# vshmyhlo/retinanet-tensorflow

Measured on AMD Instinct MI355X. Metric: train images/sec (MobileNetV2-FPN RetinaNet 512x512, bs=2/GPU), higher is better.
Workload: dtype f32

## Files before the change

include/rn_hip.h:

```cpp
#ifndef RN_HIP_H
#define RN_HIP_H

#include <stddef.h>
#include <stdint.h>

#ifdef __cplusplus
extern "C" {
#endif

typedef void* rn_stream_t;

enum rn_status {
  RN_OK = 0,
  RN_EINVAL = -1,
  RN_EUNSUPPORTED = -2,
  RN_EHIP = -3,
  RN_EWORKSPACE = -4
};

enum rn_act { RN_ACT_NONE = 0, RN_ACT_RELU = 1, RN_ACT_ELU = 2, RN_ACT_RELU6 = 3, RN_ACT_SIGMOID = 4 };
enum rn_loss_mode { RN_LOSS_BCE_DICE = 0, RN_LOSS_FOCAL = 1 };
enum rn_opt { RN_OPT_MOMENTUM = 0, RN_OPT_RMSPROP = 1, RN_OPT_ADAM = 2 };

#define RN_MAX_SEG 16

typedef struct rn_reduce_list rn_reduce_list;

#define RN_API_VERSION 421
int rn_version(void);
const char* rn_last_error(void);

void rn_same_pad(int n, int k, int s, int* out, int* pad_before);

typedef struct rn_conv_seg {
  const float* x;
  const float* wgt;
  const float* bias;
  float* y;
  const float* dy;
  float* dx;
  int32_t n, h, w;
  int32_t cout;
  int32_t x_ld;
// ... 475 lines not shown
  int32_t store_plain;
  rn_mb_rows grows;
  float* planes;
} rn_mb_gout;
size_t rn_mb_pointwise_bwd_rows(int n, int hw, int cin, int cout, int groups, rn_mb_rows* layout);
size_t rn_mb_pointwise_bwd_workspace(int n, int hw, int cin, int cout);
int rn_mb_pointwise_bwd(const float* x, const rn_mb_norm* in, const rn_mb_dy* dy, const float* w, float* dw, const rn_mb_gout* gout,
                        int n, int hw, int cin, int cout, void* workspace, size_t workspace_bytes, rn_stream_t stream,
                        rn_reduce_list* defer);
size_t rn_mb_depthwise_bwd_rows(int n, int h, int w, int c, int stride, int groups, rn_mb_rows* layout);
size_t rn_mb_depthwise_bwd_workspace(int n, int h, int w, int c, int stride);
int rn_mb_depthwise_bwd(const rn_mb_norm* in, const rn_mb_dy* dy, const float* w, float* dw, const rn_mb_gout* gout, int n, int h,
                        int wd, int stride, void* workspace, size_t workspace_bytes, rn_stream_t stream, rn_reduce_list* defer);
int rn_set_mb_dw_taps(int on);
int rn_get_mb_dw_taps(void);

int rn_iou(const float* a, int64_t na, const float* b, int64_t nb, int pairwise, float* out, int32_t* malformed,
           rn_stream_t stream);

int rn_anchor_assign(const float* boxes, const int32_t* class_ids, const int32_t* num_obj, int nimg, int max_obj,
                     const float* anchor_sizes, int num_anchors, int grid_h, int grid_w, int num_classes,
                     float* cls_out, float* reg_out, uint8_t* trainable_out, int32_t* argmax_out,
                     rn_stream_t stream);
#define RN_MAX_LEVELS 8
typedef struct rn_assign_level {
  const float* anchor_sizes;
  int grid_h, grid_w;
  float* cls_out;
  float* reg_out;
  uint8_t* trainable_out;
// ... 99 lines not shown
```

retinanet-tensorflow_amd/_rn.py:

```python
import ctypes as C
import os

import torch

_HERE = os.path.dirname(os.path.abspath(__file__))
LIB_PATH = os.environ.get("RN_LIB_PATH") or os.path.join(_HERE, "librn_hip.so")

MAX_SEG = 16
ACT = {None: 0, "none": 0, "linear": 0, "relu": 1, "elu": 2, "relu6": 3, "sigmoid": 4}
LOSS_MODE = {"bce_dice": 0, "focal": 1}
OPT = {"momentum": 0, "rmsprop": 1, "adam": 2}
OPT_BLOCK = 1024
LR_MAX_BOUNDARIES = 8
LOSS_STATS_HEADER = 8
OPT_F_NORM, OPT_F_LRDEV, OPT_F_EMA, OPT_F_CLIP, OPT_F_ACCUM, OPT_F_GATE = 1, 2, 4, 8, 16, 32
CTL_F_ACCUM, CTL_F_GUARD, CTL_F_LR, CTL_F_EMA = 1, 2, 4, 8
API_VERSION = 421


class RnError(RuntimeError):
    pass


class LrSchedule(C.Structure):
    _fields_ = [("kind", C.c_int32), ("n_boundaries", C.c_int32), ("base_lr", C.c_double), ("warmup_factor", C.c_double),
                ("final_factor", C.c_double), ("decay_factor", C.c_double), ("warmup_steps", C.c_int64), ("total_steps", C.c_int64),
                ("boundaries", C.c_int64 * LR_MAX_BOUNDARIES)]


class StepControl(C.Structure):
    _fields_ = [("features", C.c_uint32), ("optimizer_kind", C.c_int32),
                ("accumulate_steps", C.c_int32), ("micro_dev", C.c_void_p), ("accum_dev", C.c_void_p),
# ... 220 lines not shown
    "rn_group_norm_sync_bytes", "rn_group_norm_workspace", "rn_group_norm_fwd", "rn_group_norm_bwd", "rn_group_norm_plan",
    "rn_act_fwd", "rn_act_bwd", "rn_upsample_add_fwd", "rn_upsample_add_bwd_top",
    "rn_pack_weights_f16", "rn_pack_weights_f16_bytes", "rn_cast_f32_to_f16", "rn_pad_cast_rgb_f16", "rn_conv2d_fwd_f16", "rn_conv2d_f16_fold_rows", "rn_conv2d_fwd_f16_fold", "rn_group_norm_finalize", "rn_group_norm_apply_f16", "rn_group_norm_apply_res_f16", "rn_maxpool_fwd_f16", "rn_maxpool_gn_fwd_f16", "rn_upsample_add_fwd_f16",
    "rn_act_fwd_f16", "rn_flip_width", "rn_dropout", "rn_dropout_strided", "rn_maxpool_fwd", "rn_maxpool_bwd", "rn_maxpool_bwd_arg", "rn_avgpool_fwd", "rn_avgpool_bwd",
    "rn_loss_workspace", "rn_loss_fwd", "rn_loss_bwd",
    "rn_loss_terms_stats_floats", "rn_loss_terms_workspace", "rn_loss_terms_fwd", "rn_loss_terms_bwd",
    "rn_iou", "rn_anchor_assign", "rn_anchor_assign_levels", "rn_anchor_assign_levels_pair", "rn_decode_boxes", "rn_detect_workspace", "rn_detect",
    "rn_boxes_decode", "rn_nms_classwise_workspace", "rn_nms_classwise",
    "rn_optimizer_workspace", "rn_grad_norm_l2reg", "rn_optimizer_update", "rn_counter_add", "rn_add_segs",
    "rn_mb_rows_max", "rn_mb_compact_rows_layout", "rn_mb_compact_rows", "rn_mb_pointwise_rows", "rn_mb_pointwise_fwd", "rn_mb_depthwise_rows", "rn_mb_depthwise_fwd", "rn_mb_apply",
    "rn_mb_resident_sync_bytes", "rn_mb_resident_rows", "rn_mb_resident_fwd", "rn_set_product_mode", "rn_get_product_mode",
    "rn_set_x3_bfrag", "rn_get_x3_bfrag", "rn_x3_bfrag_ok", "rn_x3_bfrag_bytes", "rn_x3_pack_bfrag", "rn_gemm_batched_bfrag", "rn_conv3x3_winograd_gn_u_bytes", "rn_conv3x3_winograd_gn_weights",
    "rn_conv2d_f16_stats_tiles", "rn_group_norm_fwd_f16_tiles",
    "rn_mb_pointwise_bwd_rows", "rn_mb_pointwise_bwd_workspace", "rn_mb_pointwise_bwd",
    "rn_mb_depthwise_bwd_rows", "rn_mb_depthwise_bwd_workspace", "rn_mb_depthwise_bwd", "rn_set_mb_dw_taps", "rn_get_mb_dw_taps",
    "rn_debug_collective_standin", "rn_optimizer_norm_pairs", "rn_norm_reg_finalize",
    "rn_step_control_eval", "rn_grad_norm_partial",
    "rn_train_metrics_workspace", "rn_train_metrics_pass", "rn_train_metrics_fold", "rn_train_metrics_reset",
]


def lib():
    global _lib
    if _lib is None:
        if not os.path.exists(LIB_PATH):
            raise RnError("librn_hip.so not found at %s: build it with "
                          "`make -C retinanet-tensorflow_amd/csrc` (there is no fallback path)" % LIB_PATH)
        L = C.CDLL(LIB_PATH)
        if not hasattr(L, "rn_version") or L.rn_version() != API_VERSION:
            raise RnError("%s reports ABI version %s, these bindings need %d: rebuild it (make -C retinanet-tensorflow_amd/csrc)"
# ... 72 lines not shown
                                          C.c_void_p, C.c_size_t, C.c_void_p, C.c_void_p, C.c_void_p]
        L.rn_wino_gn_rows.argtypes = [C.c_void_p, C.c_int, C.c_int]
        L.rn_winograd_bwd_products_workspace.argtypes = [C.c_int] * 4
        L.rn_winograd_bwd_products.argtypes = [C.c_void_p] * 3 + [C.c_int] * 3 + [C.c_void_p] * 2 + [C.c_int] * 3 + \
                                              [C.c_void_p, C.c_size_t, C.c_void_p, C.c_void_p]
        L.rn_x3_bfrag_ok.argtypes = [C.c_int] * 3
        L.rn_conv2d_f16_stats_tiles.argtypes = [C.c_void_p, C.c_int, C.c_void_p, C.c_void_p]
        L.rn_group_norm_fwd_f16_tiles.argtypes = [C.c_void_p, C.c_int, C.c_void_p, C.c_void_p, C.c_void_p, C.c_void_p, C.c_void_p, C.c_void_p]
        L.rn_conv3x3_winograd_gn_u_bytes.argtypes = [C.c_int] * 3
        L.rn_conv3x3_winograd_gn_weights.argtypes = [C.c_void_p, C.c_int, C.c_int, C.c_int, C.c_void_p, C.c_size_t, C.c_void_p, C.c_void_p]
        L.rn_x3_bfrag_bytes.argtypes = [C.c_int] * 3
        L.rn_x3_pack_bfrag.argtypes = [C.c_void_p, C.c_void_p] + [C.c_int] * 4 + [C.c_void_p]
        L.rn_gemm_batched_bfrag.argtypes = [C.c_void_p] * 3 + [C.c_int] * 5 + [C.c_void_p]
        L.rn_set_x3_bfrag.argtypes = [C.c_int]
        L.rn_set_mb_dw_taps.argtypes = [C.c_int]
        L.rn_conv3x3_winograd_gn.argtypes = [C.c_void_p, C.c_int, C.c_int, C.c_int, C.c_void_p, C.c_void_p, C.c_int, C.c_void_p,
                                             C.c_void_p, C.c_size_t, C.c_void_p, C.c_void_p, C.c_void_p]
        L.rn_conv3x3_winograd_gn_bwd_wgrad.argtypes = [C.c_void_p, C.c_int, C.c_int, C.c_int, C.c_void_p, C.c_int, C.c_int, C.c_void_p, C.c_size_t,
                                                       C.c_void_p, C.c_int, C.c_void_p]
        L.rn_conv3x3_winograd_gn_bwd.argtypes = [C.c_void_p, C.c_int, C.c_int, C.c_int, C.c_void_p, C.c_void_p, C.c_int, C.c_int,
                                                 C.c_void_p, C.c_void_p, C.c_size_t, C.c_void_p, C.c_void_p, C.c_void_p]
        L.rn_conv3x3_winograd_gn_plan.argtypes = [C.c_void_p] + [C.c_int] * 6 + [C.POINTER(WinoGnPlan)]
        L.rn_group_norm_plan.argtypes = [C.c_void_p, C.c_int, C.c_void_p, C.c_int, C.c_size_t, C.POINTER(GnPlan)]
        L.rn_reduce_rows.argtypes = [C.c_void_p, C.c_void_p, C.c_int64, C.c_int, C.c_int, C.c_void_p, C.c_void_p]
        L.rn_conv2d_bias_grad.argtypes = [C.c_void_p, C.c_int, C.c_void_p, C.c_void_p, C.c_void_p, C.c_size_t,
                                          C.c_void_p, C.c_void_p]
        L.rn_group_norm_workspace.argtypes = [C.c_void_p, C.c_int, C.c_void_p]
        L.rn_group_norm_fwd.argtypes = [C.c_void_p, C.c_int, C.c_void_p, C.c_void_p, C.c_void_p, C.c_void_p,
                                        C.c_size_t, C.c_void_p]
        L.rn_group_norm_bwd.argtypes = [C.c_void_p, C.c_int, C.c_void_p, C.c_void_p, C.c_void_p, C.c_void_p,
# ... 242 lines not shown
```

retinanet-tensorflow_amd/csrc/mbconv.hip:

```cpp
#include <type_traits>

#include "mb_common.h"

namespace {


template <int BM, int BN, int WM, int WN, bool NORM, int ACT, int KS, int NST>
__global__ __launch_bounds__(WM* WN * 64 * KS) void mb_pw_fwd_kernel(const PwFwdArgs a) {
  constexpr int TG = WM * WN * 64;
  constexpr bool RES = NORM && ACT != RN_ACT_ELU && ACT != RN_ACT_RELU6 && ACT != RN_ACT_RELU;
  static_assert(TG * KS >= T || !NORM, "the prologue needs 256 threads");
  constexpr int TM = BM / WM / 32, TN = BN / WN / 32;
  constexpr int KQ = BK / 4, A_RPP = TG / KQ, A_PASS = BM / A_RPP;
  constexpr int NQ = BN / 4, B_RPP = TG / NQ, B_PASS = BK / B_RPP;
  static_assert(A_PASS >= 1 && B_PASS >= 1 && BM % A_RPP == 0 && BK % B_RPP == 0, "tile/threads mismatch");
  constexpr int OPF = BM * LDK + BK * BN;
  static_assert(KS * OPF * 4 >= (T + GMAX) * 16 && OPF >= (WM + 1) * BN * 2, "operand tiles double as scratch");
  static_assert(KS == 1 || KS * OPF >= (KS - 1) * TM * TN * 16 * TG, "operand tiles double as the split-K exchange");
  __shared__ __attribute__((aligned(16))) float smem[KS * OPF];
  __shared__ __attribute__((aligned(16))) float tab[NORM ? 2 * KMAX : 4];
  __shared__ float gstat[NORM ? GMAX : 1][2];
  const int tid = threadIdx.x, grp = tid / TG, lt = tid % TG, lane = lt & 63, wave = lt >> 6;
  float* As = smem + grp * OPF;
  float* Bs = As + BM * LDK;
// ... 359 lines not shown
                     fmaf(P.w, g.w, fmaf(R.w, y.w, Q.w)));
}

struct PwBwdArgs {
  int dbg;
  const float* x; NormDev in; int has_in;
  DyDev dy; const float* w; GoutDev go;
  int n, hw, cin, cout;
  int d_tiles_n, dblocks;
  int w_tiles_m, w_tiles_n, chunk, sps;
  float* slab;
  int wfirst;
};
constexpr int pw_lds(int pb) { return 2 * pb * LDK; }

template <int ACT_OUT, int PB, int KS, int NST>
__device__ __forceinline__ void mb_pw_dgrad_body(const PwBwdArgs& a, float* smem_all, float* tabD, float (*gstat)[2], float (*gc)[2], int blk) {
  constexpr int BM = PB, BN = PB, WM = PB / 32, WN = PB / 32, TM = 1, TN = 1, TG = WM * WN * 64;
  constexpr int KQ = BK / 4, RPP = TG / KQ, A_PASS = BM / RPP, B_PASS = BN / RPP;
  const int tid = threadIdx.x, grp = tid / TG, lt = tid % TG, lane = lt & 63, wave = lt >> 6;
  float* As = smem_all + grp * pw_lds(PB);
  float* Bs = As + BM * LDK;
  const int wm = wave / WN, wn = wave % WN;
  const int bid = rn::xcd_remap(blk, a.dblocks);
  const int tile_n = bid % a.d_tiles_n, tile_m = bid / a.d_tiles_n;
  const int KD = a.cout, ND = a.cin, M = a.n * a.hw;
  const int m0 = tile_m * BM, n0 = tile_n * BN;
  const int sample = m0 / a.hw;
  const bool plain = a.dy.dy != nullptr;
  const __amdgpu_buffer_rsrc_t ga = make_rsrc(plain ? a.dy.dy : a.dy.g, (unsigned)M * KD * 4u);
  const __amdgpu_buffer_rsrc_t ya = make_rsrc(plain ? a.dy.dy : a.dy.nd.y, (unsigned)M * KD * 4u);
// ... 29 lines not shown
  const int l31 = lane & 31, half = lane >> 5;
  const int col = n0 + wn * 32 + l31;
  const bool cok = col < ND;
  float o_mean = 0.f, o_rstd = 1.f, o_gam = 1.f, o_bet = 0.f;
  if (go.has_norm && grp == 0) {
    const int cc = cok ? col : 0, og = cc / go.nd.cpg;
    o_mean = go.nd.mean[sample * go.nd.groups + og]; o_rstd = go.nd.rstd[sample * go.nd.groups + og];
    o_gam = go.nd.gamma[cc]; o_bet = go.nd.beta[cc];
  }
#pragma unroll
  for (int st = 0; st < NST; ++st)
    if (st < nit) load_tiles(st, st);
  bool mask = false;
  uint64_t seed = 0;
  if (!plain) {
    dy_table(a.dy, sample, a.hw, 0, KD, smem_all, gstat, gc, tabD, KMAX, gpre, pre, tid);
    mask = a.dy.g_plain && a.dy.nd.drop_rate > 0.f;
    seed = a.dy.nd.seed + (a.dy.nd.seed_dev ? *a.dy.nd.seed_dev : 0ull);
  }
  if (a.dbg == 1) return;
  auto store_tiles = [&](int it, const int st) {
    const int k = (it * KS + grp) * BK + kq * 4;
#pragma unroll
    for (int i = 0; i < A_PASS; ++i) {
      float4 v = ra[st][i];
      if (!plain) {
        if (k < KD) v = dy_of(v, ry[st][i], tabD, KMAX, k, mask, a.dy.nd.drop_rate, a.dy.nd.keep_scale, seed,
                              (uint64_t)(m0 + r0 + i * RPP) * KD + k);
        else v = make_float4(0.f, 0.f, 0.f, 0.f);
      }
      *reinterpret_cast<float4*>(&As[(r0 + i * RPP) * LDK + kq * 4]) = v;
    }
#pragma unroll
    for (int j = 0; j < B_PASS; ++j) *reinterpret_cast<float4*>(&Bs[(r0 + j * RPP) * LDK + kq * 4]) = rb[st][j];
  };
  f32x16 acc[TM][TN];
  zero_acc<TM, TN>(acc);
  for (int it0 = 0; it0 < nit; it0 += NST) {
#pragma unroll
    for (int st = 0; st < NST; ++st) {
      const int it = it0 + st;
      if (it < nit) {
// ... 172 lines not shown
      const int it = it0 + st;
      if (it < nit) {
        store_tiles(it, st);
        __syncthreads();
        if (it + NST < nit) load_tiles(it + NST, st);
        if (it * KS + grp < nk) mma_ktile<BM, BN, WM, WN, true, false>(As, Bs, acc, wm, wn, lane);
        __syncthreads();
      }
    }
  }
  if (a.dbg == 2) { if (acc[0][0][0] == 123.456f) a.slab[0] = 0.f; return; }
  sum_groups<KS, 1, TG>(&acc[0][0], smem_all, grp, lt);
  if (grp == 0) store_tile<BM, BN, WM, WN>(acc, a.slab + (size_t)split * KI * NO, nullptr, m0, n0, KI, NO, NO, wm, wn, lane);
}

template <int ACT_IN, int ACT_OUT, int DPB, int DKS, int WPB, int WKS>
__global__ __launch_bounds__((DPB / 32) * (DPB / 32) * 64 * DKS) void mb_pw_bwd_kernel(const PwBwdArgs a) {
  constexpr int DTG = (DPB / 32) * (DPB / 32) * 64, WTG = (WPB / 32) * (WPB / 32) * 64;
  static_assert(DTG * DKS == WTG * WKS && DTG * DKS >= T, "both halves run in the same block size; the prologues need 256 threads");
  constexpr int LDSF = DKS * pw_lds(DPB) > WKS * pw_lds(WPB) ? DKS * pw_lds(DPB) : WKS * pw_lds(WPB);
  static_assert(LDSF * 4 >= (T + GMAX) * 16 && pw_lds(DPB) >= 3 * DPB * 2 && pw_lds(WPB) >= 2 * BK * WPB, "operand tiles double as scratch");
  static_assert((DKS == 1 || DKS * pw_lds(DPB) >= (DKS - 1) * 16 * DTG) && (WKS == 1 || WKS * pw_lds(WPB) >= (WKS - 1) * 16 * WTG),
                "operand tiles double as the split-K exchange");
  __shared__ __attribute__((aligned(16))) float smem[LDSF];
  __shared__ __attribute__((aligned(16))) float tabD[3 * KMAX];
  __shared__ __attribute__((aligned(16))) float tabA[2 * 64];
  __shared__ float gstat[GMAX][2];
  __shared__ float gc[GMAX][2];
  constexpr int NST = 1;
  const int nw = (int)gridDim.x - a.dblocks;
  const int b = (int)blockIdx.x;
  const bool is_w = a.wfirst ? b < nw : b >= a.dblocks;
  if (!is_w) mb_pw_dgrad_body<ACT_OUT, DPB, DKS, NST>(a, smem, tabD, gstat, gc, a.wfirst ? b - nw : b);
  else mb_pw_wgrad_body<(ACT_IN == -2 ? 0 : ACT_IN), WPB, WKS, NST>(a, smem, tabA, tabD, gstat, gc, a.wfirst ? b : b - a.dblocks, nw);
}

typedef float f32x4 __attribute__((ext_vector_type(4)));
struct PwBigArgs {
  int dbg;
  const float* x; NormDev in; int has_in;
  DyDev dy; const float* w; GoutDev go;
  int n, hw, cin, cout;
  int ppb, bps;
  float* slab;
};
constexpr int pw_big_lds_floats(int nti, int nto) {
  return nti * 16 * (nto * 16 + 4) + 4 * 16 * ((nto * 16 + 4) + (nti * 16 + 4));
}

template <int NTI, int NTO, bool Y_IS_A>
__global__ __launch_bounds__(T, 2) void mb_pw_bwd_big_kernel(const PwBigArgs a) {
  constexpr int CI = NTI * 16, CO = NTO * 16, SA = CI + 4, SD = CO + 4;
  constexpr int NG = (CO * 4 + 63) / 64, NA = (CI * 4 + 63) / 64;
  constexpr int NE = Y_IS_A ? 1 : 4 * NTI;
  extern __shared__ __attribute__((aligned(16))) float lds[];
  __shared__ __attribute__((aligned(16))) float tabD[3 * CO];
  __shared__ __attribute__((aligned(16))) float tabA[2 * CI];
  __shared__ __attribute__((aligned(16))) float tabO[4 * CI];
  __shared__ float gstat[GMAX][2];
  __shared__ float gc[GMAX][2];
  __shared__ __attribute__((aligned(16))) double mscratch[(T + GMAX) * 2];
  static_assert(pw_big_lds_floats(NTI, NTO) >= 2 * NTI * NTO * 256 && pw_big_lds_floats(NTI, NTO) >= 10 * CI, "the operand tiles double as the final exchange");
  constexpr bool PF = NTI * NTO < 18;
  const int tid = threadIdx.x, lane = tid & 63, wave = tid >> 6;
  const int blk = blockIdx.x, sample = blk / a.bps, bis = blk - sample * a.bps;
  const int KI = a.cin, NO = a.cout, M = a.n * a.hw;
  const int p_begin = sample * a.hw + bis * a.ppb;
  const bool plain = a.dy.dy != nullptr;
  const GoutDev& go = a.go;
  float* Wl = lds;
  float* Dt = lds + CI * SD + wave * 16 * (SD + SA);
  float* At = Dt + 16 * SD;
  const int g_r0 = (lane * 4) / NO, g_c0 = lane * 4 - g_r0 * NO, g_dr = 256 / NO, g_dc = 256 - g_dr * NO;
  const int a_r0 = (lane * 4) / KI, a_c0 = lane * 4 - a_r0 * KI, a_dr = 256 / KI, a_dc = 256 - a_dr * KI;
  auto g_slot = [&](int j, int& row, int& col) {
    row = g_r0; col = g_c0;
    for (int t = 0; t < j; ++t) { row += g_dr; col += g_dc; if (col >= NO) { col -= NO; ++row; } }
    return (lane + 64 * j) * 4 < 16 * NO;
  };
  auto a_slot = [&](int j, int& row, int& col) {
    row = a_r0; col = a_c0;
    for (int t = 0; t < j; ++t) { row += a_dr; col += a_dc; if (col >= KI) { col -= KI; ++row; } }
    return (lane + 64 * j) * 4 < 16 * KI;
  };
  const float* gsrc = plain ? a.dy.dy : a.dy.g;
  const float* ysrc = plain ? a.dy.dy : a.dy.nd.y;
  const float* asrc = a.has_in ? a.in.y : a.x;
  const bool y_sep = !Y_IS_A && go.has_norm;
  const __amdgpu_buffer_rsrc_t rg = make_rsrc(gsrc, (unsigned)M * NO * 4u);
// ... 73 lines not shown
  }
  bool mask = false, drop_in = false;
  uint64_t seed = 0, seed_in = 0;
  if (!plain) {
    dy_table(a.dy, sample, a.hw, 0, NO, mscratch, gstat, gc, tabD, CO, gp_d, pre_d, tid);
    mask = a.dy.g_plain && a.dy.nd.drop_rate > 0.f;
    seed = a.dy.nd.seed + (a.dy.nd.seed_dev ? *a.dy.nd.seed_dev : 0ull);
  }
  if (a.has_in) {
    group_stats(a.in, sample, a.hw, 0, a.in.groups, false, mscratch, gstat, gp_a, tid);
    scale_shift_table(a.in, 0, KI, 0, gstat, tabA, tabA + CI, pre_a, tid);
    drop_in = a.in.drop_rate > 0.f;
    seed_in = a.in.seed + (a.in.seed_dev ? *a.in.seed_dev : 0ull);
  }
  __syncthreads();
  f32x4 accw[NTI][NTO];
#pragma unroll
  for (int i = 0; i < NTI; ++i)
#pragma unroll
    for (int o = 0; o < NTO; ++o) accw[i][o] = f32x4{0.f, 0.f, 0.f, 0.f};
  float s1[NTI], s2[NTI];
#pragma unroll
  for (int i = 0; i < NTI; ++i) { s1[i] = 0.f; s2[i] = 0.f; }
  const NormDev& ond = go.nd;
  const bool odrop = go.has_norm && ond.drop_rate > 0.f;
  const uint64_t oseed = go.has_norm ? ond.seed + (ond.seed_dev ? *ond.seed_dev : 0ull) : 0ull;
  if (a.dbg == 1) return;
  if (PF && wave < nchunk) load_chunk(p_begin + wave * 16);
  for (int ch = wave; ch < nchunk; ch += 4) {
    const int p = p_begin + ch * 16;
    if (!PF) load_chunk(p);
#pragma unroll
    for (int j = 0; j < NG; ++j) {
      int row, col;
      if (g_slot(j, row, col)) {
        float4 v = vg[j];
        if (!plain) v = dy_of(v, vy[j], tabD, CO, col, mask, a.dy.nd.drop_rate, a.dy.nd.keep_scale, seed, (uint64_t)(p + row) * NO + col);
        *reinterpret_cast<float4*>(&Dt[row * SD + col]) = v;
      }
    }
#pragma unroll
    for (int j = 0; j < NA; ++j) {
      int row, col;
      if (a_slot(j, row, col)) {
        float4 v = va[j];
// ... 13 lines not shown
    f32x4 accd[NTI];
#pragma unroll
    for (int i = 0; i < NTI; ++i) accd[i] = f32x4{0.f, 0.f, 0.f, 0.f};
#pragma unroll 2
    for (int ks = 0; ks < NTO; ++ks) {
      const float4 a4 = *reinterpret_cast<const float4*>(&Dt[l15 * SD + 16 * ks + 4 * lq]);
      const float aa[4] = {a4.x, a4.y, a4.z, a4.w};
#pragma unroll
      for (int i = 0; i < NTI; ++i) {
        const float4 b4 = *reinterpret_cast<const float4*>(&Wl[(i * 16 + l15) * SD + 16 * ks + 4 * lq]);
        const float bb[4] = {b4.x, b4.y, b4.z, b4.w};
#pragma unroll
        for (int t = 0; t < 4; ++t) accd[i] = __builtin_amdgcn_mfma_f32_16x16x4f32(aa[t], bb[t], accd[i], 0, 0, 0);
      }
    }
#pragma unroll
    for (int t = 0; t < 4; ++t) {
      const int row = 4 * lq + t;
      float bv[NTO];
#pragma unroll
      for (int o = 0; o < NTO; ++o) bv[o] = Dt[row * SD + o * 16 + l15];
#pragma unroll
      for (int i = 0; i < NTI; ++i) {
        const int col = i * 16 + l15;
        const bool cok = col < KI;
        float av = At[row * SA + col];
        if (Y_IS_A) {
          const float raw = av;
          const float z = fmaf(raw, tabA[col], tabA[CI + col]);
          const float m = drop_in ? keep1(seed_in, (uint64_t)(p + row) * KI + col, a.in.drop_rate, a.in.keep_scale) : 1.f;
// ... 33 lines not shown
          if (!cok) outv = 0.f;
          At[row * SA + col] = outv;
        }
      }
    }
    __builtin_amdgcn_fence(__ATOMIC_RELEASE, "wavefront");
    __builtin_amdgcn_wave_barrier();
#pragma unroll
    for (int j = 0; j < NA; ++j) {
      int row, col;
      if (a_slot(j, row, col))
        *reinterpret_cast<float4*>(go.out + (size_t)p * KI + (size_t)(lane + 64 * j) * 4) = *reinterpret_cast<const float4*>(&At[row * SA + col]);
    }
    __builtin_amdgcn_fence(__ATOMIC_RELEASE, "wavefront");
    __builtin_amdgcn_wave_barrier();
  }
  if (a.dbg == 3) { if (accw[0][0][0] == 123.456f) a.slab[0] = s1[0]; return; }
  __syncthreads();
  float* ex = lds;
  auto put = [&](int slot) {
#pragma unroll
    for (int i = 0; i < NTI; ++i)
#pragma unroll
      for (int o = 0; o < NTO; ++o)
#pragma unroll
        for (int r = 0; r < 4; ++r) ex[((slot * NTI * NTO + i * NTO + o) * 4 + r) * 64 + lane] = accw[i][o][r];
  };
  auto add = [&](int slot) {
#pragma unroll
    for (int i = 0; i < NTI; ++i)
#pragma unroll
      for (int o = 0; o < NTO; ++o)
// ... 2 lines not shown
  };
  if (wave >= 2) put(wave - 2);
  __syncthreads();
  if (wave < 2) add(wave);
  __syncthreads();
  if (wave < 2) put(wave);
  __syncthreads();
  {
    float* slab = a.slab + (size_t)blk * KI * NO;
    for (int e = tid; e < NTI * NTO * 256; e += T) {
      const int ln = e & 63, r = (e >> 6) & 3, tl = e >> 8;
      const int i = tl / NTO, o = tl - i * NTO;
      const int ci = i * 16 + 4 * (ln >> 4) + r, co = o * 16 + (ln & 15);
      if (ci < KI && co < NO) slab[(size_t)ci * NO + co] = ex[((0 * NTI * NTO + tl) * 4 + r) * 64 + ln] + ex[((1 * NTI * NTO + tl) * 4 + r) * 64 + ln];
    }
  }
  if (!go.has_norm) return;
  __syncthreads();
  float* red = lds;
#pragma unroll
  for (int i = 0; i < NTI; ++i) {
    float t1 = s1[i], t2 = s2[i];
    t1 += __shfl_xor(t1, 16, 64); t1 += __shfl_xor(t1, 32, 64);
    t2 += __shfl_xor(t2, 16, 64); t2 += __shfl_xor(t2, 32, 64);
    if (lane < 16) { red[(wave * 2 + 0) * CI + i * 16 + lane] = t1; red[(wave * 2 + 1) * CI + i * 16 + lane] = t2; }
  }
  __syncthreads();
  float* chan = lds + 8 * CI;
  const int prow = sample * a.bps + bis;
  for (int c = tid; c < KI; c += T) {
// ... 520 lines not shown
  return {64, 1, 64, 1};
}
void pw_wgrad_plan(int n, int hw, int cin, int cout, int pb, int ks, int* chunk, int* sps) {
  const int tiles = rn::ceil_div(cin, pb) * rn::ceil_div(cout, pb);
  int want = rn::ceil_div(384, tiles * n);
  static const int big_blocks = getenv("RN_MB_WGRAD_BIG_BLOCKS") ? atoi(getenv("RN_MB_WGRAD_BIG_BLOCKS")) : 384;
  if (hw >= 16384 && big_blocks > 0) want = rn::ceil_div(big_blocks, tiles * n);
  if (const char* f = getenv("RN_MB_WGRAD_SPS")) { if (atoi(f) > 0) want = atoi(f); }
  const int unit = 128 * ks;
  const int units = hw % unit == 0 ? hw / unit : 1;
  int best = 1;
  for (int d = 1; d <= units && d <= want; ++d)
    if (units % d == 0) best = d;
  *sps = best; *chunk = hw / best;
}
struct PwBigCfg { int nti, nto, ppb, bps; };
bool pw_big_cfg(int n, int hw, int cin, int cout, PwBigCfg* c) {
  static const bool on = !(getenv("RN_MB_PW_BIG") && atoi(getenv("RN_MB_PW_BIG")) == 0);
  static const int min_hw = getenv("RN_MB_PW_BIG_MIN_HW") ? atoi(getenv("RN_MB_PW_BIG_MIN_HW")) : 16384;
  if (!on || hw < min_hw || hw % 64 || cin % 4 || cout % 4) return false;
  const int nti = rn::ceil_div(cin, 16), nto = rn::ceil_div(cout, 16);
  const bool built = (nti == 2 && nto == 2) || (nti == 1 && nto == 6) || (nti == 2 && nto == 9) || (nti == 2 && nto == 1) ||
                     (nti == 6 && nto == 2) || (nti == 9 && nto == 2);
  if (!built) return false;
  if (nti == 9 && hw < 65536 && !getenv("RN_MB_PW_BIG_MIN_HW")) return false;
  static const int target = getenv("RN_MB_PW_BIG_BLOCKS") ? atoi(getenv("RN_MB_PW_BIG_BLOCKS")) : 512;
  int ppb = 64;
  while ((long)n * hw / ppb > target && hw % (ppb * 2) == 0) ppb *= 2;
  while (hw / ppb > RMAX && hw % (ppb * 2) == 0) ppb *= 2;
  if (hw / ppb > RMAX) return false;
  c->nti = nti; c->nto = nto; c->ppb = ppb; c->bps = hw / ppb;
  return true;
}
struct DwBwdPlan { int th, tw, tiles_h, tiles_w, sw, nslab, oph, opw, tpb, nblk; };
bool dw_bwd_plan(int n, int h, int w, int c, int stride, int cpg, DwBwdPlan* p) {
  p->sw = dw_slab(c, cpg);
  if (!p->sw) return false;
  p->nslab = c / p->sw;
  static const int th_big = getenv("RN_MB_DWB_TH") ? atoi(getenv("RN_MB_DWB_TH")) : 8;
  static const int tw_big = getenv("RN_MB_DWB_TW") ? atoi(getenv("RN_MB_DWB_TW")) : 8;
  const bool big = (long)h * w >= 16384;
  int th = big ? th_big : 8, tw = big ? tw_big : 8;
  auto blocks = [&]() { return (long)n * rn::ceil_div(h, th) * rn::ceil_div(w, tw) * p->nslab; };
  auto too_big = [&]() { return (long)(th + 2) * (tw + 2) * (p->sw / 4) > NP * T || (long)(th / stride + 2) * (tw / stride + 2) * (p->sw / 4) > NP * T; };
  while ((blocks() < 384 && th * tw > 16) || (too_big() && th * tw > 16)) {
    if (th >= tw) th /= 2; else tw /= 2;
// ... 1 lines not shown
  p->th = th; p->tw = tw;
  p->tiles_h = rn::ceil_div(h, th); p->tiles_w = rn::ceil_div(w, tw);
  p->oph = th / stride + 2; p->opw = tw / stride + 2;
  if ((long)(th + 2) * (tw + 2) * (p->sw / 4) > NP * T || (long)p->oph * p->opw * (p->sw / 4) > NP * T) return false;
  p->tpb = dw_tiles_per_block(blocks(), p->tiles_h * p->tiles_w);
  p->nblk = rn::ceil_div(p->tiles_h * p->tiles_w, p->tpb);
  return true;
}
size_t dw_bwd_lds_bytes(const DwBwdPlan& p) {
  size_t patches = ((size_t)(p.th + 2) * (p.tw + 2) + (size_t)p.oph * p.opw) * p.sw * 4;
  size_t scratch = (size_t)(T + GMAX) * 16;
  size_t red = (size_t)(T * 44 + 2 * p.sw) * 4;
  size_t m = patches > scratch ? patches : scratch;
  return m > red ? m : red;
}
}

extern "C" size_t rn_mb_pointwise_bwd_rows(int n, int hw, int cin, int cout, int groups, rn_mb_rows* layout) {
  if (n < 1 || hw < 1 || cin < 4 || cout < 4 || groups < 1 || cin % groups || hw % 64) return 0;
  PwBigCfg big;
  if (pw_big_cfg(n, hw, cin, cout, &big)) {
    if (layout) { layout->rows_per_sample = big.bps; layout->width = groups + 1; layout->bn = big.nti * 16; }
    return (size_t)n * big.bps * (groups + 1) * 8;
  }
  const int pb = pw_bwd_cfg(n, hw, cin, cout).dpb;
  const int R = hw / pb, W = groups + rn::ceil_div(cin, pb);
  if (cin / groups > pb) return 0;
  if (layout) { layout->rows_per_sample = R; layout->width = W; layout->bn = pb; }
  return (size_t)n * R * W * 8;
}
// ... 39 lines not shown
    const size_t need = (size_t)nsplit * cin * cout * sizeof(float);
    if (workspace_bytes < need) { rn::set_error("mb pointwise bwd: workspace %zu < %zu bytes", workspace_bytes, need); return RN_EWORKSPACE; }
    b.slab = (float*)workspace;
    const bool y_is_a = a.has_in && a.go.has_norm && a.go.nd.y == a.in.y && !a.go.add1 && !a.go.add2;
    const dim3 grid((unsigned)nsplit);
    hipStream_t st = (hipStream_t)stream;
#define RN_PWBIG(NTI_, NTO_)                                                                                                    \
  do {                                                                                                                          \
    constexpr size_t lds = (size_t)pw_big_lds_floats(NTI_, NTO_) * 4;                                                           \
    static const bool attr_ = (hipFuncSetAttribute((const void*)mb_pw_bwd_big_kernel<NTI_, NTO_, true>, hipFuncAttributeMaxDynamicSharedMemorySize, (int)lds) == hipSuccess) & \
                              (hipFuncSetAttribute((const void*)mb_pw_bwd_big_kernel<NTI_, NTO_, false>, hipFuncAttributeMaxDynamicSharedMemorySize, (int)lds) == hipSuccess); \
    RN_UNSUPPORTED(!attr_, "mb pointwise bwd: %zu bytes of LDS per block refused", lds);                                                                                                                \
    if (y_is_a) hipLaunchKernelGGL((mb_pw_bwd_big_kernel<NTI_, NTO_, true>), grid, dim3(T), lds, st, b);                        \
    else hipLaunchKernelGGL((mb_pw_bwd_big_kernel<NTI_, NTO_, false>), grid, dim3(T), lds, st, b);                              \
  } while (0)
    if (big.nti == 2 && big.nto == 2) RN_PWBIG(2, 2);
    else if (big.nti == 1 && big.nto == 6) RN_PWBIG(1, 6);
    else if (big.nti == 2 && big.nto == 9) RN_PWBIG(2, 9);
    else if (big.nti == 2 && big.nto == 1) RN_PWBIG(2, 1);
    else if (big.nti == 6 && big.nto == 2) RN_PWBIG(6, 2);
    else RN_PWBIG(9, 2);
#undef RN_PWBIG
    RN_LAUNCH_CHECK();
    return rn::launch_reduce_rows((const float*)workspace, dw, (int64_t)cin * cout, nsplit, 0, st);
  }
  const PwBwdCfg cfg = pw_bwd_cfg(n, hw, cin, cout);
  a.d_tiles_n = rn::ceil_div(cin, cfg.dpb);
  a.dblocks = n * hw / cfg.dpb * a.d_tiles_n;
  a.w_tiles_m = rn::ceil_div(cin, cfg.wpb); a.w_tiles_n = rn::ceil_div(cout, cfg.wpb);
  pw_wgrad_plan(n, hw, cin, cout, cfg.wpb, cfg.wks, &a.chunk, &a.sps);
  const int nsplit = n * a.sps;
  const size_t need = (size_t)nsplit * cin * cout * sizeof(float);
  if (workspace_bytes < need) { rn::set_error("mb pointwise bwd: workspace %zu < %zu bytes", workspace_bytes, need); return RN_EWORKSPACE; }
  a.slab = nsplit == 1 ? dw : (float*)workspace;
  static const int wfirst_env = getenv("RN_MB_WGRAD_FIRST") ? atoi(getenv("RN_MB_WGRAD_FIRST")) : 1;
  a.wfirst = (wfirst_env && a.dblocks > 1024) ? 1 : 0;
  const dim3 grid((unsigned)(a.dblocks + nsplit * a.w_tiles_m * a.w_tiles_n));
  hipStream_t st = (hipStream_t)stream;
  const int act_in = in ? in->act : -2, act_out = gout->norm ? gout->norm->act : RN_ACT_NONE;
#define RN_PWB(DPB_, DKS_, WPB_, WKS_)                                                                                               \
  do {                                                                                                                               \
    constexpr int TB = (DPB_ / 32) * (DPB_ / 32) * 64 * DKS_;                                                                        \
    if (act_in == -2 && act_out == RN_ACT_NONE) hipLaunchKernelGGL((mb_pw_bwd_kernel<-2, RN_ACT_NONE, DPB_, DKS_, WPB_, WKS_>), grid, dim3(TB), 0, st, a); \
    else if (act_in == -2) hipLaunchKernelGGL((mb_pw_bwd_kernel<-2, -1, DPB_, DKS_, WPB_, WKS_>), grid, dim3(TB), 0, st, a);          \
    else if (act_in == RN_ACT_ELU && act_out == RN_ACT_ELU) hipLaunchKernelGGL((mb_pw_bwd_kernel<RN_ACT_ELU, RN_ACT_ELU, DPB_, DKS_, WPB_, WKS_>), grid, dim3(TB), 0, st, a); \
    else hipLaunchKernelGGL((mb_pw_bwd_kernel<-1, -1, DPB_, DKS_, WPB_, WKS_>), grid, dim3(TB), 0, st, a);                            \
  } while (0)
  if (cfg.dpb == 32 && cfg.dks == 8) RN_PWB(32, 8, 64, 2);
  else if (cfg.dpb == 32) RN_PWB(32, 4, 64, 1);
  else if (cfg.dks == 4) RN_PWB(64, 4, 64, 4);
  else RN_PWB(64, 1, 64, 1);
#undef RN_PWB
  RN_LAUNCH_CHECK();
  if (nsplit == 1) return RN_OK;
  return rn::launch_reduce_rows((const float*)workspace, dw, (int64_t)cin * cout, nsplit, 0, st);
}

extern "C" size_t rn_mb_depthwise_bwd_rows(int n, int h, int w, int c, int stride, int groups, rn_mb_rows* layout) {
  if (n < 1 || h < 1 || w < 1 || c < 4 || c % 4 || groups < 1 || c % groups || (stride != 1 && stride != 2)) return 0;
  DwBwdPlan p;
  if (!dw_bwd_plan(n, h, w, c, stride, c / groups, &p)) return 0;
  const int R = p.nblk;
  if (layout) { layout->rows_per_sample = R; layout->width = groups; layout->bn = c; }
// ... 89 lines not shown
```

Baseline: 493.8.

## Add split-wgrad variant of big pointwise backward kernel and shrink dgrad LDS table

Adds a SPLIT variant of the big pointwise backward kernel. Each wave accumulates the weight gradient for only a quarter of the input tiles, reading every wave's staged chunk from shared memory after a block barrier, which cuts accumulator registers and removes the cross-wave exchange at the end. The variant is gated by a split-steps setting that defaults to 0, so it stays off unless the env var or the new setter enables it. Separately, the regular pointwise backward kernel gets a template parameter that sizes the dgrad dy table to 576 channels when cout fits, shrinking static LDS to improve occupancy, and this path is on by default.

Result: no change. 498.1 (median of 6 runs) (+0.9%).

```diff
diff --git a/include/rn_hip.h b/include/rn_hip.h
--- a/include/rn_hip.h
+++ b/include/rn_hip.h
@@ -26,7 +26,7 @@
 
 typedef struct rn_reduce_list rn_reduce_list;
 
-#define RN_API_VERSION 421
+#define RN_API_VERSION 422
 int rn_version(void);
 const char* rn_last_error(void);
 
@@ -532,6 +532,8 @@
                         int wd, int stride, void* workspace, size_t workspace_bytes, rn_stream_t stream, rn_reduce_list* defer);
 int rn_set_mb_dw_taps(int on);
 int rn_get_mb_dw_taps(void);
+int rn_set_mb_pw_big_min_hw(int hw, int split_steps);
+int rn_get_mb_pw_big_min_hw(int* split_steps);
 
 int rn_iou(const float* a, int64_t na, const float* b, int64_t nb, int pairwise, float* out, int32_t* malformed,
            rn_stream_t stream);
diff --git a/retinanet-tensorflow_amd/_rn.py b/retinanet-tensorflow_amd/_rn.py
--- a/retinanet-tensorflow_amd/_rn.py
+++ b/retinanet-tensorflow_amd/_rn.py
@@ -15,7 +15,7 @@
 LOSS_STATS_HEADER = 8
 OPT_F_NORM, OPT_F_LRDEV, OPT_F_EMA, OPT_F_CLIP, OPT_F_ACCUM, OPT_F_GATE = 1, 2, 4, 8, 16, 32
 CTL_F_ACCUM, CTL_F_GUARD, CTL_F_LR, CTL_F_EMA = 1, 2, 4, 8
-API_VERSION = 421
+API_VERSION = 422
 
 
 class RnError(RuntimeError):
@@ -266,6 +266,7 @@
     "rn_conv2d_f16_stats_tiles", "rn_group_norm_fwd_f16_tiles",
     "rn_mb_pointwise_bwd_rows", "rn_mb_pointwise_bwd_workspace", "rn_mb_pointwise_bwd",
     "rn_mb_depthwise_bwd_rows", "rn_mb_depthwise_bwd_workspace", "rn_mb_depthwise_bwd", "rn_set_mb_dw_taps", "rn_get_mb_dw_taps",
+    "rn_set_mb_pw_big_min_hw", "rn_get_mb_pw_big_min_hw",
     "rn_debug_collective_standin", "rn_optimizer_norm_pairs", "rn_norm_reg_finalize",
     "rn_step_control_eval", "rn_grad_norm_partial",
     "rn_train_metrics_workspace", "rn_train_metrics_pass", "rn_train_metrics_fold", "rn_train_metrics_reset",
@@ -368,6 +369,8 @@
         L.rn_gemm_batched_bfrag.argtypes = [C.c_void_p] * 3 + [C.c_int] * 5 + [C.c_void_p]
         L.rn_set_x3_bfrag.argtypes = [C.c_int]
         L.rn_set_mb_dw_taps.argtypes = [C.c_int]
+        L.rn_set_mb_pw_big_min_hw.argtypes = [C.c_int, C.c_int]
+        L.rn_get_mb_pw_big_min_hw.argtypes = [C.POINTER(C.c_int)]
         L.rn_conv3x3_winograd_gn.argtypes = [C.c_void_p, C.c_int, C.c_int, C.c_int, C.c_void_p, C.c_void_p, C.c_int, C.c_void_p,
                                              C.c_void_p, C.c_size_t, C.c_void_p, C.c_void_p, C.c_void_p]
         L.rn_conv3x3_winograd_gn_bwd_wgrad.argtypes = [C.c_void_p, C.c_int, C.c_int, C.c_int, C.c_void_p, C.c_int, C.c_int, C.c_void_p, C.c_size_t,
diff --git a/retinanet-tensorflow_amd/csrc/mbconv.hip b/retinanet-tensorflow_amd/csrc/mbconv.hip
--- a/retinanet-tensorflow_amd/csrc/mbconv.hip
+++ b/retinanet-tensorflow_amd/csrc/mbconv.hip
@@ -397,7 +397,7 @@
 };
 constexpr int pw_lds(int pb) { return 2 * pb * LDK; }
 
-template <int ACT_OUT, int PB, int KS, int NST>
+template <int ACT_OUT, int PB, int KS, int NST, int KT>
 __device__ __forceinline__ void mb_pw_dgrad_body(const PwBwdArgs& a, float* smem_all, float* tabD, float (*gstat)[2], float (*gc)[2], int blk) {
   constexpr int BM = PB, BN = PB, WM = PB / 32, WN = PB / 32, TM = 1, TN = 1, TG = WM * WN * 64;
   constexpr int KQ = BK / 4, RPP = TG / KQ, A_PASS = BM / RPP, B_PASS = BN / RPP;
@@ -457,7 +457,7 @@
   bool mask = false;
   uint64_t seed = 0;
   if (!plain) {
-    dy_table(a.dy, sample, a.hw, 0, KD, smem_all, gstat, gc, tabD, KMAX, gpre, pre, tid);
+    dy_table(a.dy, sample, a.hw, 0, KD, smem_all, gstat, gc, tabD, KT, gpre, pre, tid);
     mask = a.dy.g_plain && a.dy.nd.drop_rate > 0.f;
     seed = a.dy.nd.seed + (a.dy.nd.seed_dev ? *a.dy.nd.seed_dev : 0ull);
   }
@@ -468,7 +468,7 @@
     for (int i = 0; i < A_PASS; ++i) {
       float4 v = ra[st][i];
       if (!plain) {
-        if (k < KD) v = dy_of(v, ry[st][i], tabD, KMAX, k, mask, a.dy.nd.drop_rate, a.dy.nd.keep_scale, seed,
+        if (k < KD) v = dy_of(v, ry[st][i], tabD, KT, k, mask, a.dy.nd.drop_rate, a.dy.nd.keep_scale, seed,
                               (uint64_t)(m0 + r0 + i * RPP) * KD + k);
         else v = make_float4(0.f, 0.f, 0.f, 0.f);
       }
@@ -671,7 +671,7 @@
   if (grp == 0) store_tile<BM, BN, WM, WN>(acc, a.slab + (size_t)split * KI * NO, nullptr, m0, n0, KI, NO, NO, wm, wn, lane);
 }
 
-template <int ACT_IN, int ACT_OUT, int DPB, int DKS, int WPB, int WKS>
+template <int ACT_IN, int ACT_OUT, int DPB, int DKS, int WPB, int WKS, int KT = KMAX>
 __global__ __launch_bounds__((DPB / 32) * (DPB / 32) * 64 * DKS) void mb_pw_bwd_kernel(const PwBwdArgs a) {
   constexpr int DTG = (DPB / 32) * (DPB / 32) * 64, WTG = (WPB / 32) * (WPB / 32) * 64;
   static_assert(DTG * DKS == WTG * WKS && DTG * DKS >= T, "both halves run in the same block size; the prologues need 256 threads");
@@ -680,7 +680,8 @@
   static_assert((DKS == 1 || DKS * pw_lds(DPB) >= (DKS - 1) * 16 * DTG) && (WKS == 1 || WKS * pw_lds(WPB) >= (WKS - 1) * 16 * WTG),
                 "operand tiles double as the split-K exchange");
   __shared__ __attribute__((aligned(16))) float smem[LDSF];
-  __shared__ __attribute__((aligned(16))) float tabD[3 * KMAX];
+  static_assert(KT >= 64 && KT <= KMAX && KT % 4 == 0, "the weight gradient's table spans 64 channels");
+  __shared__ __attribute__((aligned(16))) float tabD[3 * KT];
   __shared__ __attribute__((aligned(16))) float tabA[2 * 64];
   __shared__ float gstat[GMAX][2];
   __shared__ float gc[GMAX][2];
@@ -688,7 +689,7 @@
   const int nw = (int)gridDim.x - a.dblocks;
   const int b = (int)blockIdx.x;
   const bool is_w = a.wfirst ? b < nw : b >= a.dblocks;
-  if (!is_w) mb_pw_dgrad_body<ACT_OUT, DPB, DKS, NST>(a, smem, tabD, gstat, gc, a.wfirst ? b - nw : b);
+  if (!is_w) mb_pw_dgrad_body<ACT_OUT, DPB, DKS, NST, KT>(a, smem, tabD, gstat, gc, a.wfirst ? b - nw : b);
   else mb_pw_wgrad_body<(ACT_IN == -2 ? 0 : ACT_IN), WPB, WKS, NST>(a, smem, tabA, tabD, gstat, gc, a.wfirst ? b : b - a.dblocks, nw);
 }
 
@@ -705,9 +706,10 @@
   return nti * 16 * (nto * 16 + 4) + 4 * 16 * ((nto * 16 + 4) + (nti * 16 + 4));
 }
 
-template <int NTI, int NTO, bool Y_IS_A>
-__global__ __launch_bounds__(T, 2) void mb_pw_bwd_big_kernel(const PwBigArgs a) {
+template <int NTI, int NTO, bool Y_IS_A, bool SPLIT = false>
+__global__ __launch_bounds__(T, SPLIT ? 1 : 2) void mb_pw_bwd_big_kernel(const PwBigArgs a) {
   constexpr int CI = NTI * 16, CO = NTO * 16, SA = CI + 4, SD = CO + 4;
+  constexpr int NTW = SPLIT ? (NTI + 3) / 4 : NTI;
   constexpr int NG = (CO * 4 + 63) / 64, NA = (CI * 4 + 63) / 64;
   constexpr int NE = Y_IS_A ? 1 : 4 * NTI;
   extern __shared__ __attribute__((aligned(16))) float lds[];
@@ -728,8 +730,8 @@
   float* Wl = lds;
   float* Dt = lds + CI * SD + wave * 16 * (SD + SA);
   float* At = Dt + 16 * SD;
-  const int g_r0 = (lane * 4) / NO, g_c0 = lane * 4 - g_r0 * NO, g_dr = 256 / NO, g_dc = 256 - g_dr * NO;
-  const int a_r0 = (lane * 4) / KI, a_c0 = lane * 4 - a_r0 * KI, a_dr = 256 / KI, a_dc = 256 - a_dr * KI;
+  int g_r0 = (lane * 4) / NO, g_c0 = lane * 4 - g_r0 * NO, g_dr = 256 / NO, g_dc = 256 - g_dr * NO;
+  int a_r0 = (lane * 4) / KI, a_c0 = lane * 4 - a_r0 * KI, a_dr = 256 / KI, a_dc = 256 - a_dr * KI;
   auto g_slot = [&](int j, int& row, int& col) {
     row = g_r0; col = g_c0;
     for (int t = 0; t < j; ++t) { row += g_dr; col += g_dc; if (col >= NO) { col -= NO; ++row; } }
@@ -833,9 +835,9 @@
     seed_in = a.in.seed + (a.in.seed_dev ? *a.in.seed_dev : 0ull);
   }
   __syncthreads();
-  f32x4 accw[NTI][NTO];
-#pragma unroll
-  for (int i = 0; i < NTI; ++i)
+  f32x4 accw[NTW][NTO];
+#pragma unroll
+  for (int i = 0; i < NTW; ++i)
 #pragma unroll
     for (int o = 0; o < NTO; ++o) accw[i][o] = f32x4{0.f, 0.f, 0.f, 0.f};
   float s1[NTI], s2[NTI];
@@ -848,6 +850,9 @@
   if (PF && wave < nchunk) load_chunk(p_begin + wave * 16);
   for (int ch = wave; ch < nchunk; ch += 4) {
     const int p = p_begin + ch * 16;
+    if constexpr (SPLIT) {
+      asm volatile("" : "+v"(g_r0), "+v"(g_c0), "+v"(a_r0), "+v"(a_c0));
+    }
     if (!PF) load_chunk(p);
 #pragma unroll
     for (int j = 0; j < NG; ++j) {
@@ -891,6 +896,82 @@
         for (int t = 0; t < 4; ++t) accd[i] = __builtin_amdgcn_mfma_f32_16x16x4f32(aa[t], bb[t], accd[i], 0, 0, 0);
       }
     }
+    if constexpr (SPLIT) {
+#pragma unroll
+      for (int i = 0; i < NTI; ++i) {
+        const int col = i * 16 + l15;
+        const bool cok = col < KI;
+#pragma unroll
+        for (int r = 0; r < 4; ++r) {
+          const int row = 4 * lq + r;
+          if (Y_IS_A) {
+            const float raw = At[row * SA + col];
+            const float z = fmaf(raw, tabA[col], tabA[CI + col]);
+            const float m = drop_in ? keep1(seed_in, (uint64_t)(p + row) * KI + col, a.in.drop_rate, a.in.keep_scale) : 1.f;
+            float fa, fg;
+            if (a.in.act == RN_ACT_ELU) { const float ez = __expf(fminf(z, 0.f)); fa = z > 0.f ? z : ez - 1.f; fg = z > 0.f ? 1.f : ez; }
+            else { fa = act_of<-1>(z, a.in.act); fg = actgrad_of<-1>(z, a.in.act); }
+            const float xh = (raw - tabO[col]) * tabO[CI + col];
+            const float d = accd[i][r];
+            const float g = cok ? d * fg * m : 0.f;
+            s1[i] += g; s2[i] = fmaf(g, xh, s2[i]);
+            At[row * SA + col] = cok ? fa * m : 0.f;
+            accd[i][r] = cok ? (go.store_plain ? d : g) : 0.f;
+          } else {
+            const float d = accd[i][r] + ad[(i * 4 + r) % NE];
+            float outv = d;
+            if (go.has_norm) {
+              const float xh = (yo[(i * 4 + r) % NE] - tabO[col]) * tabO[CI + col];
+              const float z = fmaf(xh, tabO[2 * CI + col], tabO[3 * CI + col]);
+              float g = d * actgrad_of<-1>(z, ond.act);
+              if (odrop) g *= keep1(oseed, (uint64_t)(p + row) * KI + col, ond.drop_rate, ond.keep_scale);
+              if (!cok) g = 0.f;
+              s1[i] += g; s2[i] = fmaf(g, xh, s2[i]);
+              outv = go.store_plain ? d : g;
+            }
+            accd[i][r] = cok ? outv : 0.f;
+          }
+        }
+      }
+      __syncthreads();
+      const int wu = __builtin_amdgcn_readfirstlane(wave);
+#pragma unroll
+      for (int wv = 0; wv < 4; ++wv) {
+        const float* Dw = lds + CI * SD + wv * 16 * (SD + SA);
+        const float* Aw = Dw + 16 * SD;
+#pragma unroll
+        for (int t = 0; t < 4; ++t) {
+          const int row = 4 * lq + t;
+          float bv[NTO];
+#pragma unroll
+          for (int o = 0; o < NTO; ++o) bv[o] = Dw[row * SD + o * 16 + l15];
+#pragma unroll
+          for (int ii = 0; ii < NTW; ++ii) {
+            const int i = wu + 4 * ii;
+            if (i < NTI) {
+              const float av = Aw[row * SA + i * 16 + l15];
+#pragma unroll
+              for (int o = 0; o < NTO; ++o) accw[ii][o] = __builtin_amdgcn_mfma_f32_16x16x4f32(av, bv[o], accw[ii][o], 0, 0, 0);
+            }
+          }
+        }
+      }
+      __syncthreads();
+#pragma unroll
+      for (int i = 0; i < NTI; ++i)
+#pragma unroll
+        for (int r = 0; r < 4; ++r) At[(4 * lq + r) * SA + i * 16 + l15] = accd[i][r];
+      __builtin_amdgcn_fence(__ATOMIC_RELEASE, "wavefront");
+      __builtin_amdgcn_wave_barrier();
+#pragma unroll
+      for (int j = 0; j < NA; ++j) {
+        int row, col;
+        if (a_slot(j, row, col))
+          *reinterpret_cast<float4*>(go.out + (size_t)p * KI + (size_t)(lane + 64 * j) * 4) = *reinterpret_cast<const float4*>(&At[row * SA + col]);
+      }
+      __builtin_amdgcn_fence(__ATOMIC_RELEASE, "wavefront");
+      __builtin_amdgcn_wave_barrier();
+    } else {
 #pragma unroll
     for (int t = 0; t < 4; ++t) {
       const int row = 4 * lq + t;
@@ -954,8 +1035,26 @@
     }
     __builtin_amdgcn_fence(__ATOMIC_RELEASE, "wavefront");
     __builtin_amdgcn_wave_barrier();
+    }
   }
   if (a.dbg == 3) { if (accw[0][0][0] == 123.456f) a.slab[0] = s1[0]; return; }
+  if constexpr (SPLIT) {
+    float* slab = a.slab + (size_t)blk * KI * NO;
+    const int wu = __builtin_amdgcn_readfirstlane(wave);
+#pragma unroll
+    for (int ii = 0; ii < NTW; ++ii) {
+      const int i = wu + 4 * ii;
+      if (i < NTI) {
+#pragma unroll
+        for (int o = 0; o < NTO; ++o)
+#pragma unroll
+          for (int r = 0; r < 4; ++r) {
+            const int ci = i * 16 + 4 * lq + r, co = o * 16 + l15;
+            if (ci < KI && co < NO) slab[(size_t)ci * NO + co] = accw[ii][o][r];
+          }
+      }
+    }
+  } else {
   __syncthreads();
   float* ex = lds;
   auto put = [&](int slot) {
@@ -988,6 +1087,7 @@
       const int ci = i * 16 + 4 * (ln >> 4) + r, co = o * 16 + (ln & 15);
       if (ci < KI && co < NO) slab[(size_t)ci * NO + co] = ex[((0 * NTI * NTO + tl) * 4 + r) * 64 + ln] + ex[((1 * NTI * NTO + tl) * 4 + r) * 64 + ln];
     }
+  }
   }
   if (!go.has_norm) return;
   __syncthreads();
@@ -1538,22 +1638,40 @@
     if (units % d == 0) best = d;
   *sps = best; *chunk = hw / best;
 }
-struct PwBigCfg { int nti, nto, ppb, bps; };
+struct PwBigCfg { int nti, nto, ppb, bps; bool split; };
+constexpr int PW_BIG_MIN_HW = 16384, PW_SPLIT_MIN_HW = 4096, PW_SPLIT_STEPS = 0;
+int g_pw_big_min_hw = -1, g_pw_split_min_hw = -1, g_pw_split = -1;
+bool g_pw_big_env = false;
+void pw_big_defaults() {
+  if (g_pw_split >= 0) return;
+  const char* e = getenv("RN_MB_PW_BIG_MIN_HW");
+  const char* s = getenv("RN_MB_PW_BIG_SPLIT");
+  g_pw_big_env = e != nullptr;
+  g_pw_big_min_hw = e ? atoi(e) : PW_BIG_MIN_HW;
+  g_pw_split_min_hw = e ? atoi(e) : PW_SPLIT_MIN_HW;
+  g_pw_split = s ? std::max(0, atoi(s)) : PW_SPLIT_STEPS;
+}
 bool pw_big_cfg(int n, int hw, int cin, int cout, PwBigCfg* c) {
   static const bool on = !(getenv("RN_MB_PW_BIG") && atoi(getenv("RN_MB_PW_BIG")) == 0);
-  static const int min_hw = getenv("RN_MB_PW_BIG_MIN_HW") ? atoi(getenv("RN_MB_PW_BIG_MIN_HW")) : 16384;
-  if (!on || hw < min_hw || hw % 64 || cin % 4 || cout % 4) return false;
+  pw_big_defaults();
+  if (!on || hw % 64 || cin % 4 || cout % 4) return false;
   const int nti = rn::ceil_div(cin, 16), nto = rn::ceil_div(cout, 16);
-  const bool built = (nti == 2 && nto == 2) || (nti == 1 && nto == 6) || (nti == 2 && nto == 9) || (nti == 2 && nto == 1) ||
-                     (nti == 6 && nto == 2) || (nti == 9 && nto == 2);
-  if (!built) return false;
-  if (nti == 9 && hw < 65536 && !getenv("RN_MB_PW_BIG_MIN_HW")) return false;
+  const bool split = g_pw_split && hw >= g_pw_split_min_hw && hw < 65536 &&
+                     ((nti == 2 && nto == 12) || (nti == 12 && nto == 2) || (nti == 9 && nto == 2));
+  if (!split) {
+    if (hw < g_pw_big_min_hw) return false;
+    const bool built = (nti == 2 && nto == 2) || (nti == 1 && nto == 6) || (nti == 2 && nto == 9) || (nti == 2 && nto == 1) ||
+                       (nti == 6 && nto == 2) || (nti == 9 && nto == 2);
+    if (!built) return false;
+    if (nti == 9 && hw < 65536 && !g_pw_big_env) return false;
+  }
   static const int target = getenv("RN_MB_PW_BIG_BLOCKS") ? atoi(getenv("RN_MB_PW_BIG_BLOCKS")) : 512;
   int ppb = 64;
+  if (split) while (ppb < 64 * g_pw_split && hw % (ppb * 2) == 0) ppb *= 2;
   while ((long)n * hw / ppb > target && hw % (ppb * 2) == 0) ppb *= 2;
   while (hw / ppb > RMAX && hw % (ppb * 2) == 0) ppb *= 2;
   if (hw / ppb > RMAX) return false;
-  c->nti = nti; c->nto = nto; c->ppb = ppb; c->bps = hw / ppb;
+  c->nti = nti; c->nto = nto; c->ppb = ppb; c->bps = hw / ppb; c->split = split;
   return true;
 }
 struct DwBwdPlan { int th, tw, tiles_h, tiles_w, sw, nslab, oph, opw, tpb, nblk; };
@@ -1585,6 +1703,20 @@
   size_t m = patches > scratch ? patches : scratch;
   return m > red ? m : red;
 }
+}
+
+extern "C" int rn_set_mb_pw_big_min_hw(int hw, int split_steps) {
+  RN_CHECK_ARG(hw >= 64 && split_steps >= 0 && split_steps <= 64, "rn_set_mb_pw_big_min_hw: hw %d (>= 64), split_steps %d (0 .. 64)", hw, split_steps);
+  g_pw_split = split_steps;
+  g_pw_big_env = false;
+  if (split_steps == 0) { g_pw_big_min_hw = hw; g_pw_split_min_hw = PW_SPLIT_MIN_HW; }
+  else { g_pw_big_min_hw = PW_BIG_MIN_HW; g_pw_split_min_hw = hw; }
+  return RN_OK;
+}
+extern "C" int rn_get_mb_pw_big_min_hw(int* split_steps) {
+  pw_big_defaults();
+  if (split_steps) *split_steps = g_pw_split;
+  return g_pw_split ? g_pw_split_min_hw : g_pw_big_min_hw;
 }
 
 extern "C" size_t rn_mb_pointwise_bwd_rows(int n, int hw, int cin, int cout, int groups, rn_mb_rows* layout) {
@@ -1654,13 +1786,26 @@
     if (y_is_a) hipLaunchKernelGGL((mb_pw_bwd_big_kernel<NTI_, NTO_, true>), grid, dim3(T), lds, st, b);                        \
     else hipLaunchKernelGGL((mb_pw_bwd_big_kernel<NTI_, NTO_, false>), grid, dim3(T), lds, st, b);                              \
   } while (0)
-    if (big.nti == 2 && big.nto == 2) RN_PWBIG(2, 2);
+#define RN_PWSPLIT(NTI_, NTO_)                                                                                                  \
+  do {                                                                                                                          \
+    constexpr size_t lds = (size_t)pw_big_lds_floats(NTI_, NTO_) * 4;                                                           \
+    static const bool attr_ = (hipFuncSetAttribute((const void*)mb_pw_bwd_big_kernel<NTI_, NTO_, true, true>, hipFuncAttributeMaxDynamicSharedMemorySize, (int)lds) == hipSuccess) & \
+                              (hipFuncSetAttribute((const void*)mb_pw_bwd_big_kernel<NTI_, NTO_, false, true>, hipFuncAttributeMaxDynamicSharedMemorySize, (int)lds) == hipSuccess); \
+    RN_UNSUPPORTED(!attr_, "mb pointwise bwd: %zu bytes of LDS per block refused", lds);                                        \
+    if (y_is_a) hipLaunchKernelGGL((mb_pw_bwd_big_kernel<NTI_, NTO_, true, true>), grid, dim3(T), lds, st, b);                  \
+    else hipLaunchKernelGGL((mb_pw_bwd_big_kernel<NTI_, NTO_, false, true>), grid, dim3(T), lds, st, b);                        \
+  } while (0)
+    if (big.split && big.nti == 2) RN_PWSPLIT(2, 12);
+    else if (big.split && big.nti == 12) RN_PWSPLIT(12, 2);
+    else if (big.split) RN_PWSPLIT(9, 2);
+    else if (big.nti == 2 && big.nto == 2) RN_PWBIG(2, 2);
     else if (big.nti == 1 && big.nto == 6) RN_PWBIG(1, 6);
     else if (big.nti == 2 && big.nto == 9) RN_PWBIG(2, 9);
     else if (big.nti == 2 && big.nto == 1) RN_PWBIG(2, 1);
     else if (big.nti == 6 && big.nto == 2) RN_PWBIG(6, 2);
     else RN_PWBIG(9, 2);
 #undef RN_PWBIG
+#undef RN_PWSPLIT
     RN_LAUNCH_CHECK();
     return rn::launch_reduce_rows((const float*)workspace, dw, (int64_t)cin * cout, nsplit, 0, st);
   }
@@ -1678,15 +1823,17 @@
   const dim3 grid((unsigned)(a.dblocks + nsplit * a.w_tiles_m * a.w_tiles_n));
   hipStream_t st = (hipStream_t)stream;
   const int act_in = in ? in->act : -2, act_out = gout->norm ? gout->norm->act : RN_ACT_NONE;
-#define RN_PWB(DPB_, DKS_, WPB_, WKS_)                                                                                               \
+#define RN_PWB(DPB_, DKS_, WPB_, WKS_, ...)                                                                                            \
   do {                                                                                                                               \
     constexpr int TB = (DPB_ / 32) * (DPB_ / 32) * 64 * DKS_;                                                                        \
-    if (act_in == -2 && act_out == RN_ACT_NONE) hipLaunchKernelGGL((mb_pw_bwd_kernel<-2, RN_ACT_NONE, DPB_, DKS_, WPB_, WKS_>), grid, dim3(TB), 0, st, a); \
-    else if (act_in == -2) hipLaunchKernelGGL((mb_pw_bwd_kernel<-2, -1, DPB_, DKS_, WPB_, WKS_>), grid, dim3(TB), 0, st, a);          \
-    else if (act_in == RN_ACT_ELU && act_out == RN_ACT_ELU) hipLaunchKernelGGL((mb_pw_bwd_kernel<RN_ACT_ELU, RN_ACT_ELU, DPB_, DKS_, WPB_, WKS_>), grid, dim3(TB), 0, st, a); \
-    else hipLaunchKernelGGL((mb_pw_bwd_kernel<-1, -1, DPB_, DKS_, WPB_, WKS_>), grid, dim3(TB), 0, st, a);                            \
+    if (act_in == -2 && act_out == RN_ACT_NONE) hipLaunchKernelGGL((mb_pw_bwd_kernel<-2, RN_ACT_NONE, DPB_, DKS_, WPB_, WKS_, ##__VA_ARGS__>), grid, dim3(TB), 0, st, a); \
+    else if (act_in == -2) hipLaunchKernelGGL((mb_pw_bwd_kernel<-2, -1, DPB_, DKS_, WPB_, WKS_, ##__VA_ARGS__>), grid, dim3(TB), 0, st, a);          \
+    else if (act_in == RN_ACT_ELU && act_out == RN_ACT_ELU) hipLaunchKernelGGL((mb_pw_bwd_kernel<RN_ACT_ELU, RN_ACT_ELU, DPB_, DKS_, WPB_, WKS_, ##__VA_ARGS__>), grid, dim3(TB), 0, st, a); \
+    else hipLaunchKernelGGL((mb_pw_bwd_kernel<-1, -1, DPB_, DKS_, WPB_, WKS_, ##__VA_ARGS__>), grid, dim3(TB), 0, st, a);                            \
   } while (0)
-  if (cfg.dpb == 32 && cfg.dks == 8) RN_PWB(32, 8, 64, 2);
+  static const bool small_tab = !(getenv("RN_MB_PW_SMALL_TAB") && atoi(getenv("RN_MB_PW_SMALL_TAB")) == 0);
+  if (cfg.dpb == 32 && cfg.dks == 8 && cout <= 576 && small_tab) RN_PWB(32, 8, 64, 2, 576);
+  else if (cfg.dpb == 32 && cfg.dks == 8) RN_PWB(32, 8, 64, 2);
   else if (cfg.dpb == 32) RN_PWB(32, 4, 64, 1);
   else if (cfg.dks == 4) RN_PWB(64, 4, 64, 4);
   else RN_PWB(64, 1, 64, 1);
```
